# bayesiains/nflows

Hardware: AMD Instinct MI355X
Metric: log_prob samples/sec (dim=64, K=8, 32-layer RQ-NSF) + max |fwd∘inv − x| (higher is better)
Workload: dtype f32 (inputs, outputs, spline arithmetic, accumulation; conditioner GEMMs: every fp32 operand carried as 3 f16 pieces = 33 significand bits, i.e. at the reference's own fp32 operand width, 5 cross products per multiply-add -- 3 on the f16 MFMA, the 2 at the 2^-22 level from the pieces' high bytes on

## Files before the change

### include/nflows_amd.h

```cpp
#ifndef NFLOWS_AMD_H
#define NFLOWS_AMD_H

#include <stddef.h>
#include <stdint.h>

#ifdef __cplusplus
extern "C" {
#endif

#define NFA_ABI_VERSION 19

#define NFA_OK 0
#define NFA_ERR_INVALID_ARGUMENT 1
#define NFA_ERR_UNSUPPORTED 2
#define NFA_ERR_MIN_BIN_WIDTH 3
#define NFA_ERR_MIN_BIN_HEIGHT 4
#define NFA_ERR_HIP 5

#define NFA_STATUS_OUTSIDE_DOMAIN 1
#define NFA_STATUS_NEG_DISCRIMINANT 2
#define NFA_STATUS_BAD_INDEX 4

#define NFA_FLAG_INVERSE 1
#define NFA_FLAG_ACCUMULATE_LOGABSDET 2
// ... 3 lines not shown

#define NFA_FLAG_STANDARD_NORMAL_LOG_PROB 16
#define NFA_FLAG_SKIP_OUTPUTS 32

#define NFA_FLAG_RESIDUAL_BLOCKS 64
#define NFA_FLAG_PAD_COLUMNS_SHIFT 8
#define NFA_FLAG_PAD_COLUMNS_MASK 0x700
#define NFA_FLAG_PAD_COLUMNS(n) ((n) << NFA_FLAG_PAD_COLUMNS_SHIFT)
#define NFA_FLAG_ACTIVATION_SHIFT 12
#define NFA_FLAG_ACTIVATION_MASK 0x7000
#define NFA_ACTIVATION_RELU 0
#define NFA_ACTIVATION_LEAKY_RELU 1
#define NFA_ACTIVATION_ELU 2
#define NFA_ACTIVATION_TANH 3
#define NFA_FLAG_ACTIVATION(a) ((a) << NFA_FLAG_ACTIVATION_SHIFT)

#define NFA_TAILS_NONE 0
#define NFA_TAILS_LINEAR 1

#define NFA_SCALE_DEFAULT 0
#define NFA_SCALE_GENERAL 1
#define NFA_SCALE_ADDITIVE 2
#define NFA_SCALE_GIVEN 3
#define NFA_SCALE_SOFTPLUS 4

typedef struct nfa_rqs_spec {
    int32_t num_bins;
    int32_t tails;
    double left, right;
    double bottom, top;
// ... 361 lines not shown
```

### nflows_amd/_native.py

```python
import ctypes
import os

import torch

_PKG_DIR = os.path.dirname(os.path.abspath(__file__))
LIB_PATH = os.environ.get("NFLOWS_AMD_LIB") or os.path.join(_PKG_DIR, "libnflows_amd.so")

OK = 0
ERR_INVALID_ARGUMENT = 1
ERR_UNSUPPORTED = 2
ERR_MIN_BIN_WIDTH = 3
ERR_MIN_BIN_HEIGHT = 4
ERR_HIP = 5

STATUS_OUTSIDE_DOMAIN = 1
STATUS_NEG_DISCRIMINANT = 2
STATUS_BAD_INDEX = 4

FLAG_INVERSE, FLAG_ACCUMULATE_LOGABSDET, FLAG_WEIGHTS_BF16X3, FLAG_LOGITS_LOG2E = 1, 2, 4, 8
FLAG_STANDARD_NORMAL_LOG_PROB, FLAG_SKIP_OUTPUTS = 16, 32
FLAG_RESIDUAL_BLOCKS = 64
FLAG_PAD_COLUMNS_SHIFT = 8
FLAG_ACTIVATION_SHIFT = 12
ACTIVATION_RELU, ACTIVATION_LEAKY_RELU, ACTIVATION_ELU, ACTIVATION_TANH = 0, 1, 2, 3
TAILS_NONE, TAILS_LINEAR = 0, 1
NONLIN_EXP, NONLIN_TANH, NONLIN_LOG_TANH, NONLIN_LEAKY_RELU, NONLIN_SIGMOID, NONLIN_CAUCHY_CDF = 0, 1, 2, 3, 4, 5
SCALE_DEFAULT, SCALE_GENERAL, SCALE_ADDITIVE, SCALE_GIVEN, SCALE_SOFTPLUS = 0, 1, 2, 3, 4

ABI_VERSION = 19

EXPORTS = (
    "nfa_abi_version",
    "nfa_build_arch",
    "nfa_strerror",
    "nfa_last_hip_error",
    "nfa_rqs_coupling_f32",
    "nfa_rqs_coupling_backward_f32",
    "nfa_rqs_coupling_fused_linear_f32",
# ... 328 lines not shown
```

### nflows_amd/csrc/f16x3_gemm.hpp

```cpp
#pragma once

#include "bf16x3_gemm.hpp"

namespace nfa {

typedef _Float16 f16x8 __attribute__((ext_vector_type(8)));
typedef int i32x8 __attribute__((ext_vector_type(8)));

namespace k8x {

constexpr int kScaleA = 119, kScaleB = 127;

#ifdef NFA_ABL_NO_MFMA
#define NFA_K8X_F16(a, b, c) (c)
#define NFA_K8X_BF8(a, b, c) (c)
#else
#define NFA_K8X_F16(a, b, c) __builtin_amdgcn_mfma_f32_32x32x16_f16(a, b, c, 0, 0, 0)
#define NFA_K8X_BF8(a, b, c) __builtin_amdgcn_mfma_scale_f32_32x32x64_f8f6f4(a, b, c, 1, 1, 0, kScaleA, 0, kScaleB)
#endif

__device__ __forceinline__ void request_stage(WeightStream& sm) {
    const int dst_slot = sm.slot >= 1 ? sm.slot - 1 : kRing - 1;
    const char* stage = reinterpret_cast<const char*>(sm.w) + (size_t)sm.fetch * (kStageVec4 * 16);
    const __amdgpu_buffer_rsrc_t rsrc =
        __builtin_amdgcn_make_buffer_rsrc(const_cast<char*>(stage), (short)0, kStageVec4 * 16, 0x00020000);
    const int wave = __builtin_amdgcn_readfirstlane(sm.tid >> 6);
    char* slot = reinterpret_cast<char*>(sm.ring) + dst_slot * (kStageVec4 * 16) + wave * (kWave * 16);
    const unsigned lane_off = (unsigned)sm.tid * 16u;
#pragma unroll
    for (int i = 0; i < 3; ++i)
        __builtin_amdgcn_raw_ptr_buffer_load_lds(rsrc, (__attribute__((address_space(3))) void*)(slot + i * kBlock * 16), 16,
                                                 lane_off, i * kBlock * 16, 0, 0);
    sm.fetch = (sm.fetch + 1 == sm.num_stages) ? 0 : sm.fetch + 1;
}

struct Pieces {
    uvec4 h, l, r;
};

#define NFA_K8X_ASM asm volatile

#define NFA_K8X_SPLIT_REST                                                  \
    "v_fma_mixlo_f16 %1, %3, 1.0, 0 op_sel_hi:[0,0,0]\n\t"                  \
    "v_fma_mixhi_f16 %1, %4, 1.0, 0 op_sel_hi:[0,0,0]\n\t"                  \
    "v_fma_mix_f32 %3, %3, 1.0, -%1 op_sel_hi:[0,0,1]\n\t"                  \
    "v_fma_mix_f32 %4, %4, 1.0, -%1 op_sel:[0,0,1] op_sel_hi:[0,0,1]\n\t"   \
    "v_fma_mixlo_f16 %2, %3, %8, 0 op_sel_hi:[0,0,0]\n\t"                   \
    "v_fma_mixhi_f16 %2, %4, %8, 0 op_sel_hi:[0,0,0]"
// ... 78 lines not shown

__device__ __forceinline__ i32x8 join_x(vec4f lo, vec4f hi) {
    const uvec4 a = __builtin_bit_cast(uvec4, lo), b = __builtin_bit_cast(uvec4, hi);
    return i32x8{(int)a[0], (int)a[1], (int)a[2], (int)a[3], (int)b[0], (int)b[1], (int)b[2], (int)b[3]};
}

struct Lead {
    vec4f h0, l0, h1, l1;
};
__device__ __forceinline__ Lead read_lead(const vec4f* stage) {
    return Lead{stage[0 * 64], stage[1 * 64], stage[2 * 64], stage[3 * 64]};
}

#define NFA_K8X_FENCE() __builtin_amdgcn_sched_barrier(0)

template <bool LAST>
__device__ __forceinline__ void stage_kmajor(f32x16& acc0, f32x16& acc1, const Pieces& b0, const Pieces& b1, const i32x8& bx,
                                             WeightStream& sm, int lane, Lead& lead) {
    request_stage(sm);
    const vec4f* cur = sm.ring + sm.slot * kStageVec4 + lane;
    const f16x8 bh0 = __builtin_bit_cast(f16x8, b0.h), bl0 = __builtin_bit_cast(f16x8, b0.l);
    const f16x8 bh1 = __builtin_bit_cast(f16x8, b1.h), bl1 = __builtin_bit_cast(f16x8, b1.l);
    const vec4f x0l = cur[4 * 64], x0h = cur[5 * 64];
    const vec4f h0 = cur[6 * 64], l0 = cur[7 * 64], h1 = cur[8 * 64], l1 = cur[9 * 64], x1l = cur[10 * 64], x1h = cur[11 * 64];
    NFA_K8X_FENCE();
    {
        const f16x8 ah0 = __builtin_bit_cast(f16x8, lead.h0), al0 = __builtin_bit_cast(f16x8, lead.l0);
        const f16x8 ah1 = __builtin_bit_cast(f16x8, lead.h1), al1 = __builtin_bit_cast(f16x8, lead.l1);
        acc0 = NFA_K8X_F16(ah0, bl0, acc0);
        acc0 = NFA_K8X_F16(al0, bh0, acc0);
        acc0 = NFA_K8X_F16(ah0, bh0, acc0);
        acc0 = NFA_K8X_F16(ah1, bl1, acc0);
        acc0 = NFA_K8X_F16(al1, bh1, acc0);
        acc0 = NFA_K8X_F16(ah1, bh1, acc0);
        acc0 = NFA_K8X_BF8(join_x(x0l, x0h), bx, acc0);
    }
    const f16x8 ah0 = __builtin_bit_cast(f16x8, h0), al0 = __builtin_bit_cast(f16x8, l0);
    const f16x8 ah1 = __builtin_bit_cast(f16x8, h1), al1 = __builtin_bit_cast(f16x8, l1);
    const i32x8 ax = join_x(x1l, x1h);
    acc1 = NFA_K8X_F16(ah0, bl0, acc1);
    acc1 = NFA_K8X_F16(al0, bh0, acc1);
    acc1 = NFA_K8X_F16(ah0, bh0, acc1);
    NFA_K8X_FENCE();
    stream_advance(sm);
    if constexpr (!LAST) lead = read_lead(sm.ring + sm.slot * kStageVec4 + lane);
    NFA_K8X_FENCE();
    acc1 = NFA_K8X_F16(ah1, bl1, acc1);
    acc1 = NFA_K8X_F16(al1, bh1, acc1);
    acc1 = NFA_K8X_F16(ah1, bh1, acc1);
    acc1 = NFA_K8X_BF8(ax, bx, acc1);
}

template <int NKS, class PairFn>
__device__ __forceinline__ void gemm_kmajor_pairs(f32x16 (&acc)[4], WeightStream& sm, int lane, PairFn&& pair) {
    static_assert(NKS % 2 == 0, "pairs of k-steps");
    Lead lead = read_lead(sm.ring + sm.slot * kStageVec4 + lane);
#pragma unroll
    for (int pr = 0; pr < NKS / 2; ++pr) {
        Pieces b0, b1;
        pair(pr, b0, b1);
        const i32x8 bx = bf8_operand(b0, b1);
        stage_kmajor<false>(acc[0], acc[1], b0, b1, bx, sm, lane, lead);
        if (pr + 1 < NKS / 2) stage_kmajor<false>(acc[2], acc[3], b0, b1, bx, sm, lane, lead);
        else stage_kmajor<true>(acc[2], acc[3], b0, b1, bx, sm, lane, lead);
    }
}

template <int NKS>
__device__ __forceinline__ void gemm_kmajor(f32x16 (&acc)[4], const Pieces (&p)[8], WeightStream& sm, int lane) {
    gemm_kmajor_pairs<NKS>(acc, sm, lane, [&](int pr, Pieces& b0, Pieces& b1) {
        b0 = p[2 * pr];
        b1 = p[2 * pr + 1];
    });
}

__device__ __forceinline__ void gemm_kmajor_relu(f32x16 (&acc)[4], const f32x16 (&src)[4], float scale, WeightStream& sm,
                                                 int lane) {
    gemm_kmajor_pairs<8>(acc, sm, lane, [&](int pr, Pieces& b0, Pieces& b1) {
        if (pr == 0) tile_to_pieces<true, true>(src[pr], scale, b0, b1);
        else tile_to_pieces<true, false>(src[pr], scale, b0, b1);
    });
}

}
}
```

### nflows_amd/csrc/rqs_resnet_f16x3.hip

```cpp

#include "rqs_resnet_f16x3_kernel.hpp"

using namespace nfa;

static k8x::KernelFn f16x3_kernel(bool inverse, int init_ks, int K, bool dbg, bool bias_lds) {
    if (K != 8) {
        const k8x::KernelFn kern = k8x::bins_kernel_a(K, inverse, init_ks, bias_lds);
        return kern ? kern : k8x::bins_kernel_b(K, inverse, init_ks, bias_lds);
    }
    if (!bias_lds) {
        if (init_ks == 4)
            return dbg ? (inverse ? k8x::rqs_resnet_f16x3_global_bias_kernel<true, 4, true> : k8x::rqs_resnet_f16x3_global_bias_kernel<false, 4, true>)
                       : (inverse ? k8x::rqs_resnet_f16x3_global_bias_kernel<true, 4> : k8x::rqs_resnet_f16x3_global_bias_kernel<false, 4>);
        return dbg ? (inverse ? k8x::rqs_resnet_f16x3_global_bias_kernel<true, 2, true> : k8x::rqs_resnet_f16x3_global_bias_kernel<false, 2, true>)
                   : (inverse ? k8x::rqs_resnet_f16x3_global_bias_kernel<true, 2> : k8x::rqs_resnet_f16x3_global_bias_kernel<false, 2>);
    }
    if (init_ks == 4)
        return dbg ? (inverse ? k8x::rqs_resnet_f16x3_kernel<true, 4, true> : k8x::rqs_resnet_f16x3_kernel<false, 4, true>)
                   : (inverse ? k8x::rqs_resnet_f16x3_kernel<true, 4> : k8x::rqs_resnet_f16x3_kernel<false, 4>);
    return dbg ? (inverse ? k8x::rqs_resnet_f16x3_kernel<true, 2, true> : k8x::rqs_resnet_f16x3_kernel<false, 2, true>)
               : (inverse ? k8x::rqs_resnet_f16x3_kernel<true, 2> : k8x::rqs_resnet_f16x3_kernel<false, 2>);
}

static int launch_f16x3(const LayerCall& c, const float* scales, float act_scale, float* dbg_logits = nullptr) {
    int exponent = 0;
    if (!(act_scale > 0.0f) || frexpf(act_scale, &exponent) != 0.5f) return NFA_ERR_INVALID_ARGUMENT;
    k8x::Args a;
    int activation = 0;
    int rc = check_layer_call(c, {NFA_FLAG_ACTIVATION_MASK, true, false, false}, &a.sp, &activation);
    if (rc != NFA_OK) return rc;
    if (activation != NFA_ACTIVATION_RELU || (dbg_logits && a.sp.K != 8)) return NFA_ERR_UNSUPPORTED;
    if (c.batch == 0) return NFA_OK;
    if (!layer_buffers_given(c) || !c.bias || !scales || !c.redo) return NFA_ERR_INVALID_ARGUMENT;
    rc = fill_layer_args(a, c);
    if (rc != NFA_OK) return rc;
    a.act_scale = act_scale;
    a.bias = c.bias;
    a.scales = scales;
    a.tables = c.tables;
    a.redo = c.redo;
    a.dbg_logits = dbg_logits;
    const int init_ks = c.num_identity > 32 ? 4 : 2;
    const int rows_per_feature = spline_rows_per_feature(a.sp.K);
    a.num_stages = init_ks + 16 * c.num_blocks + 2 * (c.num_transform * rows_per_feature / 32);
    a.bias_per_layer = 128 + 256 * c.num_blocks + c.num_transform * rows_per_feature;
    const size_t lds_rows = (size_t)kRing * kStageVec4 * 16 + (size_t)(kBlock / kWave) * c.features * kRowPad * sizeof(float);
    const int final_floats = c.num_transform * rows_per_feature;
    const size_t lds_area = lds_rows + (size_t)k8x::bias_area_floats(c.num_blocks, final_floats) * sizeof(float);
    const size_t lds_plain = lds_rows + (size_t)final_floats * sizeof(float);
    const size_t two_per_cu = 80 * 1024 - 2048;
    const size_t launch_limit = kCuLds - 2048;
    const bool bias_lds = lds_area <= launch_limit && (dbg_logits || lds_area <= two_per_cu || lds_plain > two_per_cu);
    const size_t lds = bias_lds ? lds_area : lds_plain;
    int64_t blocks = c.batch >> 7;
    const int64_t per_cu = lds <= two_per_cu ? 2 : 1;
    const int64_t cap = (int64_t)device_cu_count() * per_cu;
    if (blocks > cap) blocks = cap;
    const bool inv = (c.flags & NFA_FLAG_INVERSE) != 0;
    const k8x::KernelFn kern = f16x3_kernel(inv, init_ks, a.sp.K, dbg_logits, bias_lds);
    if (!kern) return NFA_ERR_UNSUPPORTED;
    note_layer_kernel("k8x::rqs_resnet_f16x3_kernel<inverse=%d, init_ks=%d, K=%d, dbg=%d, bias=%s>", inv ? 1 : 0, init_ks, a.sp.K,
                      dbg_logits ? 1 : 0, bias_lds ? "lds" : "global");
    return launch_kernel(kern, dim3((unsigned)blocks), dim3(kBlock), lds, (hipStream_t)c.stream, a, kCuLds - 2048);
}

extern "C" int nfa_rqs_flow_resnet_f16x3_f32(const float* inputs, const void* weights_packed, const float* bias_packed,
                                             const float* scales, const int32_t* flow_tables, int32_t num_layers,
                                             float* outputs, float* logabsdet, int32_t* redo_blocks, int32_t* status,
                                             int64_t batch, int32_t features, int32_t num_transform,
                                             int32_t num_identity, int32_t hidden_features, int32_t num_blocks,
                                             float act_scale, const nfa_rqs_spec* spec, int32_t flags, void* stream) {
    return launch_f16x3({inputs, weights_packed, bias_packed, flow_tables, num_layers, outputs, logabsdet, redo_blocks,
                         status, batch, features, num_transform, num_identity, hidden_features, num_blocks, spec, flags,
// ... 19 lines not shown
```

### nflows_amd/csrc/rqs_resnet_f16x3_kernel.hpp

```cpp
#pragma once

#include "f16x3_gemm.hpp"
#include "rqs_resnet_f16_kernel.hpp"

#include <hip/hip_ext.h>
#include <stdlib.h>
#include <type_traits>

namespace nfa {
namespace k8x {

struct Args {
    const float* x;
    const vec4f* w;
    const float* bias;
    const float* scales;
    const int32_t* tables;
    float* out;
    float* lad;
    int32_t* redo;
    int32_t* status;
    int64_t batch;
    int D, dt, di, num_blocks, num_layers, num_stages, bias_per_layer, accumulate;
    RqsDev sp;
// ... 81 lines not shown
        k8h::spline_seq_range<MASK, (U0 * N) / 32, (U1 * N) / 32>(f, sp);
    }
};

#define NFA_K8X_PUMP_F16(U, A_, B_)                                         \
    acc = NFA_K8X_F16(A_, B_, acc);                                         \
    __builtin_amdgcn_sched_barrier(0);                                      \
    w.template span<(U), (U) + 1>();                                        \
    __builtin_amdgcn_sched_barrier(0)
#define NFA_K8X_PUMP_BF8(U, A_, B_)                                         \
    acc = NFA_K8X_BF8(A_, B_, acc);                                         \
    __builtin_amdgcn_sched_barrier(0);                                      \
    w.template span<(U), (U) + 2>();                                        \
    __builtin_amdgcn_sched_barrier(0)

template <int HS, class W>
__device__ __forceinline__ void stage_pumped(f32x16& acc, const Pieces (&p)[8], const i32x8 (&bx)[4], WeightStream& sm, int lane,
                                             Lead& lead, W& w) {
    request_stage(sm);
    const vec4f* cur = sm.ring + sm.slot * kStageVec4 + lane;
    vec4f xa = cur[8 * 64], xb = cur[9 * 64];
    vec4f fh0 = lead.h0, fl0 = lead.l0, fh1 = lead.h1, fl1 = lead.l1;
    {
        const Pieces& b0 = p[HS * 4 + 0];
        const Pieces& b1 = p[HS * 4 + 1];
        const f16x8 bh0 = __builtin_bit_cast(f16x8, b0.h), bl0 = __builtin_bit_cast(f16x8, b0.l);
        const f16x8 bh1 = __builtin_bit_cast(f16x8, b1.h), bl1 = __builtin_bit_cast(f16x8, b1.l);
        const f16x8 ah0 = __builtin_bit_cast(f16x8, fh0), al0 = __builtin_bit_cast(f16x8, fl0);
        const f16x8 ah1 = __builtin_bit_cast(f16x8, fh1), al1 = __builtin_bit_cast(f16x8, fl1);
        const i32x8 ax = join_x(xa, xb);
        NFA_K8X_PUMP_F16(HS * 16 + 0, ah0, bl0);
        NFA_K8X_PUMP_F16(HS * 16 + 1, al0, bh0);
        NFA_K8X_PUMP_F16(HS * 16 + 2, ah0, bh0);
        fh0 = cur[4 * 64];
// ... 9 lines not shown
    }
    {
        const Pieces& b0 = p[HS * 4 + 2];
        const Pieces& b1 = p[HS * 4 + 3];
        const f16x8 bh0 = __builtin_bit_cast(f16x8, b0.h), bl0 = __builtin_bit_cast(f16x8, b0.l);
        const f16x8 bh1 = __builtin_bit_cast(f16x8, b1.h), bl1 = __builtin_bit_cast(f16x8, b1.l);
        const f16x8 ah0 = __builtin_bit_cast(f16x8, fh0), al0 = __builtin_bit_cast(f16x8, fl0);
        const f16x8 ah1 = __builtin_bit_cast(f16x8, fh1), al1 = __builtin_bit_cast(f16x8, fl1);
        const i32x8 ax = join_x(xa, xb);
        NFA_K8X_PUMP_F16(HS * 16 + 8, ah0, bl0);
        NFA_K8X_PUMP_F16(HS * 16 + 9, al0, bh0);
        NFA_K8X_PUMP_F16(HS * 16 + 10, ah0, bh0);
        NFA_K8X_PUMP_F16(HS * 16 + 11, ah1, bl1);
        NFA_K8X_PUMP_F16(HS * 16 + 12, al1, bh1);
        NFA_K8X_PUMP_F16(HS * 16 + 13, ah1, bh1);
        stream_advance(sm);
        lead = read_lead(sm.ring + sm.slot * kStageVec4 + lane);
        __builtin_amdgcn_sched_barrier(0);
        NFA_K8X_PUMP_BF8(HS * 16 + 14, ax, bx[HS * 2 + 1]);
    }
}
#undef NFA_K8X_PUMP_F16
#undef NFA_K8X_PUMP_BF8

template <class W>
__device__ __forceinline__ void gemm_tile_pumped(f32x16& acc, const Pieces (&p)[8], const i32x8 (&bx)[4], WeightStream& sm, int lane,
                                                 Lead& lead, W&& w) {
    stage_pumped<0>(acc, p, bx, sm, lane, lead, w);
    stage_pumped<1>(acc, p, bx, sm, lane, lead, w);
}

template <int TI, int T, int KB, class Steps, class BiasPtr>
__device__ __forceinline__ void any_group_tiles(f32x16& acc, Steps& f, BiasPtr gb, const Pieces (&p)[8], const i32x8 (&bx)[4],
                                                WeightStream& sm, int lane, Lead& lead, const RqsDev& sp) {
    if constexpr (TI < T) {
        constexpr int kMask = k8h::any_tile_mask(KB, TI);
        load_bias_tile(acc, gb + TI * 32);
        if constexpr (kMask != 0) gemm_tile_pumped(acc, p, bx, sm, lane, lead, SeqWeave<kMask, Steps>{f, sp});
        else gemm_tile_pumped(acc, p, bx, sm, lane, lead, NoWeave{});
        k8h::take_chunk<TI, KB>(f, acc);
        any_group_tiles<TI + 1, T, KB, Steps, BiasPtr>(acc, f, gb, p, bx, sm, lane, lead, sp);
    }
}

__device__ __forceinline__ bool not_finite(float v) { return !(__builtin_fabsf(v) < INFINITY); }

template <bool INVERSE, int INIT_KS, bool DBG, int KB, bool BIAS_LDS>
__device__ __forceinline__ void rqs_resnet_f16x3_body(const Args& a) {
    static_assert(!DBG || KB == 8, "the diagnostic instances: 8 bins");
    constexpr int kFinalRows = KB == 8 ? 24 : 16 * ((3 * KB - 1 + 15) / 16);
    constexpr int NW = kBlock / kWave;
    extern __shared__ __attribute__((aligned(16))) float lds_dyn[];
    __shared__ int s_tab[2][kTabLayer];
    __shared__ int s_final[128];
    __shared__ int s_bad[NW];
    const int tid = threadIdx.x, lane = tid & 63, wave = __builtin_amdgcn_readfirstlane(tid >> 6);
    const int D = a.D, dt = a.dt;
    int my_status = 0;
    auto checked = [&](int v, bool used) {
        my_status |= (used && (v < 0 || v >= D)) ? NFA_STATUS_BAD_INDEX : 0;
        return v < 0 ? 0 : (v >= D ? D - 1 : v);
    };
    const int te = tid & (kTabLayer - 1);
    s_tab[0][te] = checked(a.tables[te], te < kTabTr ? te < a.di : te - kTabTr < dt);
    s_final[te] = checked(a.tables[a.num_layers * kTabLayer + te], te < D);

    WeightStream sm;
    sm.w = a.w;
    sm.ring = reinterpret_cast<vec4f*>(lds_dyn);
    sm.slot = 1;
    sm.fetch = 0;
    sm.num_stages = a.num_stages * a.num_layers;
    sm.tid = tid;
    lds_f32* s_area = (lds_f32*)lds_dyn + kRing * kStageVec4 * 4 + NW * D * kRowPad;
    lds_f32* s_traw = s_area + bias_area_hidden_floats(a.num_blocks);
    auto request_hidden = [&](int layer) {
        const float* src = a.bias + (size_t)layer * a.bias_per_layer;
        const int bytes = bias_area_hidden_floats(a.num_blocks) * 4;
        if (wave >= 2) bias_area_piece<4>(src, bytes, (wave - 2) * 256, s_area + (wave - 2) * 64);
        for (int j = wave; j < a.num_blocks; j += NW) bias_area_piece<16>(src, bytes, 512 + j * 1024, s_area + 128 + j * 256);
    };
    if constexpr (BIAS_LDS) request_hidden(0);
    request_stage(sm);
    sm.slot = 2;
    request_stage(sm);
    sm.slot = 0;
    asm volatile("s_waitcnt vmcnt(0)" ::: "memory");
    __syncthreads();

#ifdef NFA_K8X_STAGGER
    if (blockIdx.x >= (gridDim.x >> 1))
        for (int i = 0; i < NFA_K8X_STAGGER; ++i) __builtin_amdgcn_s_sleep(127);
#endif
    lds_f32* s_row = (lds_f32*)lds_dyn + kRing * kStageVec4 * 4 + wave * D * kRowPad;
    lds_f32* s_fbias = BIAS_LDS ? s_traw + kTabLayer : s_area;
    auto request_final = [&](int layer) {
        const float* src = a.bias + (size_t)layer * a.bias_per_layer + bias_area_hidden_floats(a.num_blocks);
        const int bytes = dt * kFinalRows * 4;
        for (int j = wave; j * 1024 < bytes; j += NW) bias_area_piece<16>(src, bytes, j * 1024, s_fbias + j * 256);
    };
    auto request_table = [&](int layer) {
        if (wave < 2) bias_area_piece<4>(a.tables + layer * kTabLayer, kTabLayer * 4, wave * 256, s_traw + wave * 64);
    };
    const int groups = dt >> 2;
    const int64_t num_quads = a.batch >> 7;
    const int gemms = 2 + 2 * a.num_blocks;
    const float S = a.act_scale;
    int tb = 0;

    for (int64_t quad = blockIdx.x; quad < num_quads; quad += gridDim.x) {
        const int64_t row0 = (quad << 7) + (wave << 5);
        int lane_here = lane, di = a.di;
        asm volatile("" : "+v"(lane_here), "+s"(di));
        const int half = lane_here >> 5, r = lane_here & 31;
        {
            const vec4f* xv = reinterpret_cast<const vec4f*>(a.x + row0 * D);
            const int nvec = D * 8;
            for (int e0 = lane; e0 < nvec; e0 += kWave * 4) {
                vec4f v[4];
#pragma unroll
                for (int u = 0; u < 4; ++u) {
                    const int e = e0 + u * kWave;
                    v[u] = xv[e < nvec ? e : 0];
                }
#pragma unroll
                for (int u = 0; u < 4; ++u) {
// ... 2 lines not shown
                        const int rr = (e * 4) / D, c0 = e * 4 - rr * D;
                        s_row[(c0 + 0) * kRowPad + rr] = v[u].x;
                        s_row[(c0 + 1) * kRowPad + rr] = v[u].y;
                        s_row[(c0 + 2) * kRowPad + rr] = v[u].z;
                        s_row[(c0 + 3) * kRowPad + rr] = v[u].w;
                    }
                }
            }
        }
        __builtin_amdgcn_fence(__ATOMIC_RELEASE, "wavefront");
        __builtin_amdgcn_fence(__ATOMIC_ACQUIRE, "wavefront");

        float lad_acc = 0.0f;
        int quad_status = 0;
        for (int layer = 0; layer < a.num_layers; ++layer) {
            if ((layer + (blockIdx.x >= (gridDim.x >> 1) ? 1 : 0)) & 1) __builtin_amdgcn_s_setprio(1);
            else __builtin_amdgcn_s_setprio(0);
            const int* tab = s_tab[tb];
            const int nl = layer + 1 < a.num_layers ? layer + 1 : 0;
            if constexpr (!BIAS_LDS) {
                unsigned all = ~0u;
                asm volatile("" : "+s"(all));
                const int te_l = (int)__builtin_amdgcn_mbcnt_hi(all, __builtin_amdgcn_mbcnt_lo(all, 0u)) + ((wave & 1) << 6);
                s_tab[tb ^ 1][te_l] = checked(a.tables[nl * kTabLayer + te_l], te_l < kTabTr ? te_l < a.di : te_l - kTabTr < dt);
            }
            if constexpr (BIAS_LDS) {
                request_final(layer);
                request_table(nl);
                __builtin_amdgcn_sched_barrier(0);
            }
            std::conditional_t<BIAS_LDS, const lds_f32*, const float*> bias;
            if constexpr (BIAS_LDS) bias = s_area + half * 16;
// ... 10 lines not shown
                    v0 = i0 < di ? v0 : 0.0f;
                    v1 = i0 + 1 < di ? v1 : 0.0f;
                    unsigned hi, lo, rr;
                    split3_scaled(v0, v1, S, hi, lo, rr);
                    p[ks].h[j2] = hi;
                    p[ks].l[j2] = lo;
                    p[ks].r[j2] = rr;
                }
            }

            f32x16 h[4];
            float hs;
            {
#pragma unroll
                for (int t = 0; t < 4; ++t) load_bias_tile(h[t], bias + t * 32);
                gemm_kmajor<INIT_KS>(h, p, sm, lane);
                float s0[2];
                uniform_load(sc, s0);
                hs = s0[0];
            }
            bias += 128;
            sc += 2;
            if constexpr (BIAS_LDS) {
                unsigned all = ~0u;
                asm volatile("" : "+s"(all));
                const int te_l = (int)__builtin_amdgcn_mbcnt_hi(all, __builtin_amdgcn_mbcnt_lo(all, 0u)) + ((wave & 1) << 6);
                s_tab[tb ^ 1][te_l] = checked(((const lds_i32*)s_traw)[te_l], te_l < kTabTr ? te_l < a.di : te_l - kTabTr < dt);
            } else {
                const float* fbias = a.bias + (size_t)layer * a.bias_per_layer + 128 + 256 * a.num_blocks;
                for (int i = tid; i < dt * kFinalRows; i += kBlock) s_fbias[i] = fbias[i];
                if (a.num_blocks == 0) __syncthreads();
            }

            for (int blk = 0; blk < a.num_blocks; ++blk) {
                float sb[4];
                f32x16 u[4];
#pragma unroll
                for (int t = 0; t < 4; ++t) load_bias_tile(u[t], bias + t * 32);
                gemm_kmajor_relu(u, h, hs, sm, lane);
                uniform_load(sc, sb);
                const float skip = hs * sb[3];
#pragma unroll
                for (int t = 0; t < 4; ++t) {
                    f32x16 b1;
                    load_bias_tile(b1, bias + 128 + t * 32);
#pragma unroll
                    for (int q_ = 0; q_ < 16; ++q_) h[t][q_] = __builtin_fmaf(h[t][q_], skip, b1[q_]);
                }
                gemm_kmajor_relu(h, u, sb[0], sm, lane);
                hs = sb[2];
                bias += 256;
                sc += 4;
            }

            if constexpr (BIAS_LDS) {
                request_hidden(nl);
                __builtin_amdgcn_sched_barrier(0);
            }
#pragma unroll
            for (int t = 0; t < 4; ++t) tile_to_pieces<false>(h[t], hs, p[2 * t], p[2 * t + 1]);

            if constexpr (KB == 8) {
                using Steps = FusedSteps<INVERSE, 8>;
                Steps fa{}, fb{};
// ... 21 lines not shown
                            float* dst = a.dbg_logits + (size_t)(row0 + r) * (dt * kFinalRows) + tile * 32 + half * 16;
#pragma unroll
                            for (int q_ = 0; q_ < 16; ++q_) dst[q_] = t[q_] * kappa;
                            asm volatile("s_waitcnt vmcnt(0)" ::: "memory");
                        }
                    }
                };
                UnitWeave<k8h::kUnitNumA, Steps> w0{fa, fb, a.sp};
                UnitWeave<k8h::kUnitFinishA, Steps> w1{fa, fb, a.sp};
                UnitWeave<k8h::kUnitFinishB, Steps> w2{fa, fb, a.sp};
                for (int g = 0; g < groups; ++g) {
                    lds_f32* slot0 = s_row + tab[kTabTr + g * 4 + half * 2] * kRowPad + r;
                    lds_f32* slot1 = s_row + tab[kTabTr + g * 4 + half * 2 + 1] * kRowPad + r;
                    load_bias_tile(acc[0], fbias + (g * 3 + 0) * 32);
                    if (g > 0) {
                        gemm_tile_pumped(acc[0], p, bx, sm, lane, lead, w2);
                        commit(fb, slot_b);
                    } else {
                        gemm_tile_pumped(acc[0], p, bx, sm, lane, lead, NoWeave{});
                    }
                    store_logits(acc[0], g * 3 + 0);
                    fa.x = *slot0;
#pragma unroll
                    for (int j = 0; j < 8; ++j) {
                        fa.ew[j] = acc[0][j];
                        fa.eh[j] = acc[0][8 + j];
                    }
                    load_bias_tile(acc[1], fbias + (g * 3 + 1) * 32);
                    gemm_tile_pumped(acc[1], p, bx, sm, lane, lead, w0);
                    store_logits(acc[1], g * 3 + 1);
                    fb.x = *slot1;
#pragma unroll
                    for (int j = 0; j < 8; ++j) {
                        if (j < 7) fa.sd[j] = acc[1][j];
                        fb.ew[j] = acc[1][8 + j];
                    }
                    load_bias_tile(acc[2], fbias + (g * 3 + 2) * 32);
                    gemm_tile_pumped(acc[2], p, bx, sm, lane, lead, w1);
                    store_logits(acc[2], g * 3 + 2);
                    commit(fa, slot0);
#pragma unroll
                    for (int j = 0; j < 8; ++j) {
                        fb.eh[j] = acc[2][j];
                        if (j < 7) fb.sd[j] = acc[2][8 + j];
                    }
                    slot_b = slot1;
                }
                k8h::spline_unit_range<k8h::kUnitFinishB, 0, k8h::spline_unit_slices<k8h::kUnitFinishB, Steps>()>(fa, fb, a.sp);
                commit(fb, slot_b);
            }
            else {
                constexpr int T = kFinalRows / 16;
                static_assert(T >= 1 && T <= 6, "2 .. 32 bins");
// ... 37 lines not shown
            }
            tb ^= 1;
            __builtin_amdgcn_fence(__ATOMIC_RELEASE, "wavefront");
            __builtin_amdgcn_fence(__ATOMIC_ACQUIRE, "wavefront");
        }

        lad_acc += __shfl_xor(lad_acc, 32, kWave);
        const float sumsq = tile_row_sumsq((const float*)s_row, a.Ds, half, r);
        const bool bad = not_finite(lad_acc) || not_finite(sumsq);
        const bool wave_bad = __builtin_amdgcn_ballot_w64(bad) != 0;
        if (lane == 0) s_bad[wave] = wave_bad ? 1 : 0;
        asm volatile("s_waitcnt vmcnt(0)" ::: "memory");
        __syncthreads();
        int any_bad = 0;
#pragma unroll
        for (int w_ = 0; w_ < NW; ++w_) any_bad |= s_bad[w_];
        if (!any_bad) {
            if (!a.skip_out) {
                vec4f* ov = reinterpret_cast<vec4f*>(a.out + row0 * D);
                const int nvec = D * 8;
                for (int e = lane; e < nvec; e += kWave) {
                    const int rr = (e * 4) / D, c0 = e * 4 - rr * D;
                    vec4f v;
                    v.x = s_row[s_final[c0 + 0] * kRowPad + rr];
                    v.y = s_row[s_final[c0 + 1] * kRowPad + rr];
                    v.z = s_row[s_final[c0 + 2] * kRowPad + rr];
                    v.w = s_row[s_final[c0 + 3] * kRowPad + rr];
                    ov[e] = v;
                }
            }
            if (half == 0) {
                float* dst = a.lad + row0 + r;
                float v = a.accumulate ? *dst + lad_acc : lad_acc;
                if (a.normal) v = (-0.5f * sumsq - a.log_z) + v;
                *dst = v;
            }
            my_status |= quad_status;
        }
        if (tid == 0) a.redo[quad] = any_bad ? 1 : 0;
        asm volatile("s_waitcnt vmcnt(0)" ::: "memory");
        __syncthreads();
    }
    asm volatile("s_waitcnt vmcnt(0)" ::: "memory");
    if (my_status && a.status) atomicOr(a.status, my_status);
}

template <bool INVERSE, int INIT_KS, bool DBG = false, int KB = 8>
__global__ void __launch_bounds__(kBlock, 2) rqs_resnet_f16x3_kernel(const Args a) {
    rqs_resnet_f16x3_body<INVERSE, INIT_KS, DBG, KB, true>(a);
}
template <bool INVERSE, int INIT_KS, bool DBG = false, int KB = 8>
__global__ void __launch_bounds__(kBlock, 2) rqs_resnet_f16x3_global_bias_kernel(const Args a) {
    rqs_resnet_f16x3_body<INVERSE, INIT_KS, DBG, KB, false>(a);
}

}
}


namespace nfa {
namespace k8x {
typedef void (*KernelFn)(const Args);
KernelFn bins_kernel_a(int K, bool inverse, int init_ks, bool bias_lds);
KernelFn bins_kernel_b(int K, bool inverse, int init_ks, bool bias_lds);
}
}
```

### nflows_amd/ops.py

```python
import ctypes
import math
import os

import numpy as np
import torch

from . import _native as N
from . import autograd as AG
from .errors import InputOutsideDomain

_status_words = {}
_error_mode = "deferred"
_launch_hook = None


_last_redo = None


def last_redo_blocks():
    return None if _last_redo is None else int((_last_redo != 0).sum().item())


def set_launch_hook(hook):
    global _launch_hook
# ... 2045 lines not shown


_ACTIVATION_CODES = {id(torch.nn.functional.relu): N.ACTIVATION_RELU, id(torch.relu): N.ACTIVATION_RELU,
                     id(torch.nn.functional.leaky_relu): N.ACTIVATION_LEAKY_RELU, id(torch.nn.functional.elu): N.ACTIVATION_ELU,
                     id(torch.tanh): N.ACTIVATION_TANH, id(torch.nn.functional.tanh): N.ACTIVATION_TANH}


def activation_code(fn):
    return _ACTIVATION_CODES.get(id(fn))


K8S_ENABLED = os.environ.get("NFA_K8S", "1") != "0"
K8S_ALWAYS = os.environ.get("NFA_K8S", "1") == "2"
K8C_ENABLED = os.environ.get("NFA_K8C", "1") != "0"
K8C_ALWAYS = os.environ.get("NFA_K8C", "1") == "2"
_cu_counts = {}


def use_tile16(batch, num_bins, context, device, activation=0):
    if not K8S_ENABLED or num_bins != 8 or context is not None or activation != N.ACTIVATION_RELU:
        return 0
    if capture_last_layer_logits.active is not None:
        return 0
    key = device.index if device.index is not None else torch.cuda.current_device()
    cus = _cu_counts.get(key)
    if cus is None:
        cus = _cu_counts[key] = torch.cuda.get_device_properties(key).multi_processor_count
    if K8C_ENABLED and capture_last_layer_bins.active is None and (K8C_ALWAYS or (batch + 95) // 96 <= cus):
        return 2
    return 1 if (K8S_ALWAYS or (batch + 127) // 128 <= cus) else 0
# ... 189 lines not shown
    def finish(self, redo):
        self.logits = unpack_last_layer_logits(self._packed, self._dt)
        self.redo = redo


def rqs_coupling_resnet_f16x3(inputs, packed_f16x3, packed_exact, tables, num_transform, num_identity, num_blocks,
                              spec, inverse=False, accumulate_into=None, num_layers=1,
                              standard_normal_log_prob=False, pad=None, act_scale=K8X_ACT_SCALE):
    weights, biases, scales = packed_f16x3

    def launch(x, ctx, out, lad, redo, flags, status, stream):
        lib = N.load()
        B, D = x.shape
        args = (N.ptr(x), N.ptr(weights), N.ptr(biases), N.ptr(scales), N.ptr(tables), num_layers, N.ptr(out),
                N.ptr(lad), N.ptr(redo), status, B, D, num_transform, num_identity, 128, num_blocks,
                float(act_scale), ctypes.byref(spec), flags, stream)
        capture = capture_last_layer_logits.active
        if capture is None:
            return lib.nfa_rqs_flow_resnet_f16x3_f32(*args)
        rc = lib.nfa_rqs_flow_resnet_f16x3_logits_f32(*args, N.ptr(capture.buffer(B, num_transform, x.device)))
        if rc == N.OK:
            capture.finish(redo)
        return rc
    return _whole_layer_launch(launch, inputs, inverse, accumulate_into, standard_normal_log_prob, pad, spec=spec,
                               redo=(*packed_exact, tables, num_layers, num_transform, num_identity, num_blocks))


def rqs_coupling_fused_linear(inputs, hidden, weight_packed, bias_padded, transform_idx, spec,
                              inverse=False, in_perm=None, out_scatter=None, accumulate_into=None):
    N.require_device_f32("inputs", inputs, 2)
    N.require_device_f32("hidden", hidden, 2)
# ... 29 lines not shown
```

Baseline: 26.74 million.

## Add wide 8-wave k8x resnet kernel sharing one weight stream across two quads

Adds a wide form of the f16x3 resnet flow kernel with 512 threads (8 waves) per block. Each block processes two 128-row quads at once, and both halves share a double-width LDS weight ring, so every streamed weight stage is fetched once for two quads instead of once per block. The form is chosen automatically when the batch is large enough (at least 2 blocks per CU), with an environment and flag override. The cost is double the LDS ring size, one block per CU, barriers that now span 8 waves, and predicated handling of an odd trailing quad.

```diff
diff --git a/include/nflows_amd.h b/include/nflows_amd.h
--- a/include/nflows_amd.h
+++ b/include/nflows_amd.h
@@ -41,6 +41,12 @@
 #define NFA_ACTIVATION_ELU 2
 #define NFA_ACTIVATION_TANH 3
 #define NFA_FLAG_ACTIVATION(a) ((a) << NFA_FLAG_ACTIVATION_SHIFT)
+#define NFA_FLAG_K8X_FORM_SHIFT 16
+#define NFA_FLAG_K8X_FORM_MASK 0x30000
+#define NFA_K8X_FORM_AUTO 0
+#define NFA_K8X_FORM_NARROW 1
+#define NFA_K8X_FORM_WIDE 2
+#define NFA_FLAG_K8X_FORM(f) ((f) << NFA_FLAG_K8X_FORM_SHIFT)
 
 #define NFA_TAILS_NONE 0
 #define NFA_TAILS_LINEAR 1
diff --git a/nflows_amd/_native.py b/nflows_amd/_native.py
--- a/nflows_amd/_native.py
+++ b/nflows_amd/_native.py
@@ -22,6 +22,7 @@
 FLAG_RESIDUAL_BLOCKS = 64
 FLAG_PAD_COLUMNS_SHIFT = 8
 FLAG_ACTIVATION_SHIFT = 12
+FLAG_K8X_FORM_SHIFT = 16
 ACTIVATION_RELU, ACTIVATION_LEAKY_RELU, ACTIVATION_ELU, ACTIVATION_TANH = 0, 1, 2, 3
 TAILS_NONE, TAILS_LINEAR = 0, 1
 NONLIN_EXP, NONLIN_TANH, NONLIN_LOG_TANH, NONLIN_LEAKY_RELU, NONLIN_SIGMOID, NONLIN_CAUCHY_CDF = 0, 1, 2, 3, 4, 5
diff --git a/nflows_amd/csrc/f16x3_gemm.hpp b/nflows_amd/csrc/f16x3_gemm.hpp
--- a/nflows_amd/csrc/f16x3_gemm.hpp
+++ b/nflows_amd/csrc/f16x3_gemm.hpp
@@ -32,6 +32,36 @@
         __builtin_amdgcn_raw_ptr_buffer_load_lds(rsrc, (__attribute__((address_space(3))) void*)(slot + i * kBlock * 16), 16,
                                                  lane_off, i * kBlock * 16, 0, 0);
     sm.fetch = (sm.fetch + 1 == sm.num_stages) ? 0 : sm.fetch + 1;
+}
+
+template <int WAVES, int SUB>
+__device__ __forceinline__ void request_stage(WeightStream& sm) {
+    static_assert(WAVES == 4 || WAVES == 8, "narrow or wide");
+    if constexpr (WAVES == 4) {
+        request_stage(sm);
+    } else if constexpr (SUB == 0) {
+        const int dst_half = sm.slot >= 2 ? sm.slot - 2 : sm.slot + 2 * kRing - 2;
+        const char* stage = reinterpret_cast<const char*>(sm.w) + (size_t)sm.fetch * (kStageVec4 * 16);
+        const __amdgpu_buffer_rsrc_t rsrc =
+            __builtin_amdgcn_make_buffer_rsrc(const_cast<char*>(stage), (short)0, 2 * kStageVec4 * 16, 0x00020000);
+        const int wave = __builtin_amdgcn_readfirstlane(sm.tid >> 6);
+        char* slot = reinterpret_cast<char*>(sm.ring) + dst_half * (kStageVec4 * 16) + wave * (kWave * 16);
+        const unsigned lane_off = (unsigned)sm.tid * 16u;
+#pragma unroll
+        for (int i = 0; i < 3; ++i)
+            __builtin_amdgcn_raw_ptr_buffer_load_lds(rsrc, (__attribute__((address_space(3))) void*)(slot + i * WAVES * kWave * 16),
+                                                     16, lane_off, i * WAVES * kWave * 16, 0, 0);
+        sm.fetch = (sm.fetch + 2 == sm.num_stages) ? 0 : sm.fetch + 2;
+    }
+}
+template <int WAVES, int SUB>
+__device__ __forceinline__ void stream_advance(WeightStream& sm) {
+    if constexpr (WAVES == 4) {
+        stream_advance(sm);
+    } else {
+        if constexpr (SUB == 1) asm volatile("s_waitcnt vmcnt(3)\n\ts_waitcnt lgkmcnt(0)\n\ts_barrier" ::: "memory");
+        sm.slot = (sm.slot + 1 == 2 * kRing) ? 0 : sm.slot + 1;
+    }
 }
 
 struct Pieces {
@@ -140,10 +170,10 @@
 
 #define NFA_K8X_FENCE() __builtin_amdgcn_sched_barrier(0)
 
-template <bool LAST>
+template <bool LAST, int WAVES = 4, int SUB = 0>
 __device__ __forceinline__ void stage_kmajor(f32x16& acc0, f32x16& acc1, const Pieces& b0, const Pieces& b1, const i32x8& bx,
                                              WeightStream& sm, int lane, Lead& lead) {
-    request_stage(sm);
+    request_stage<WAVES, SUB>(sm);
     const vec4f* cur = sm.ring + sm.slot * kStageVec4 + lane;
     const f16x8 bh0 = __builtin_bit_cast(f16x8, b0.h), bl0 = __builtin_bit_cast(f16x8, b0.l);
     const f16x8 bh1 = __builtin_bit_cast(f16x8, b1.h), bl1 = __builtin_bit_cast(f16x8, b1.l);
@@ -168,7 +198,7 @@
     acc1 = NFA_K8X_F16(al0, bh0, acc1);
     acc1 = NFA_K8X_F16(ah0, bh0, acc1);
     NFA_K8X_FENCE();
-    stream_advance(sm);
+    stream_advance<WAVES, SUB>(sm);
     if constexpr (!LAST) lead = read_lead(sm.ring + sm.slot * kStageVec4 + lane);
     NFA_K8X_FENCE();
     acc1 = NFA_K8X_F16(ah1, bl1, acc1);
@@ -177,7 +207,7 @@
     acc1 = NFA_K8X_BF8(ax, bx, acc1);
 }
 
-template <int NKS, class PairFn>
+template <int NKS, int WAVES, class PairFn>
 __device__ __forceinline__ void gemm_kmajor_pairs(f32x16 (&acc)[4], WeightStream& sm, int lane, PairFn&& pair) {
     static_assert(NKS % 2 == 0, "pairs of k-steps");
     Lead lead = read_lead(sm.ring + sm.slot * kStageVec4 + lane);
@@ -186,23 +216,24 @@
         Pieces b0, b1;
         pair(pr, b0, b1);
         const i32x8 bx = bf8_operand(b0, b1);
-        stage_kmajor<false>(acc[0], acc[1], b0, b1, bx, sm, lane, lead);
-        if (pr + 1 < NKS / 2) stage_kmajor<false>(acc[2], acc[3], b0, b1, bx, sm, lane, lead);
-        else stage_kmajor<true>(acc[2], acc[3], b0, b1, bx, sm, lane, lead);
-    }
-}
-
-template <int NKS>
+        stage_kmajor<false, WAVES, 0>(acc[0], acc[1], b0, b1, bx, sm, lane, lead);
+        if (pr + 1 < NKS / 2) stage_kmajor<false, WAVES, 1>(acc[2], acc[3], b0, b1, bx, sm, lane, lead);
+        else stage_kmajor<true, WAVES, 1>(acc[2], acc[3], b0, b1, bx, sm, lane, lead);
+    }
+}
+
+template <int NKS, int WAVES = 4>
 __device__ __forceinline__ void gemm_kmajor(f32x16 (&acc)[4], const Pieces (&p)[8], WeightStream& sm, int lane) {
-    gemm_kmajor_pairs<NKS>(acc, sm, lane, [&](int pr, Pieces& b0, Pieces& b1) {
+    gemm_kmajor_pairs<NKS, WAVES>(acc, sm, lane, [&](int pr, Pieces& b0, Pieces& b1) {
         b0 = p[2 * pr];
         b1 = p[2 * pr + 1];
     });
 }
 
+template <int WAVES = 4>
 __device__ __forceinline__ void gemm_kmajor_relu(f32x16 (&acc)[4], const f32x16 (&src)[4], float scale, WeightStream& sm,
                                                  int lane) {
-    gemm_kmajor_pairs<8>(acc, sm, lane, [&](int pr, Pieces& b0, Pieces& b1) {
+    gemm_kmajor_pairs<8, WAVES>(acc, sm, lane, [&](int pr, Pieces& b0, Pieces& b1) {
         if (pr == 0) tile_to_pieces<true, true>(src[pr], scale, b0, b1);
         else tile_to_pieces<true, false>(src[pr], scale, b0, b1);
     });
diff --git a/nflows_amd/csrc/rqs_resnet_f16x3.hip b/nflows_amd/csrc/rqs_resnet_f16x3.hip
--- a/nflows_amd/csrc/rqs_resnet_f16x3.hip
+++ b/nflows_amd/csrc/rqs_resnet_f16x3.hip
@@ -22,13 +22,20 @@
                : (inverse ? k8x::rqs_resnet_f16x3_kernel<true, 2> : k8x::rqs_resnet_f16x3_kernel<false, 2>);
 }
 
+static k8x::KernelFn f16x3_wide_kernel(bool inverse, int init_ks) {
+    if (init_ks == 4) return inverse ? k8x::rqs_resnet_f16x3_kernel_wide<true, 4> : k8x::rqs_resnet_f16x3_kernel_wide<false, 4>;
+    return inverse ? k8x::rqs_resnet_f16x3_kernel_wide<true, 2> : k8x::rqs_resnet_f16x3_kernel_wide<false, 2>;
+}
+
 static int launch_f16x3(const LayerCall& c, const float* scales, float act_scale, float* dbg_logits = nullptr) {
     int exponent = 0;
     if (!(act_scale > 0.0f) || frexpf(act_scale, &exponent) != 0.5f) return NFA_ERR_INVALID_ARGUMENT;
     k8x::Args a;
     int activation = 0;
-    int rc = check_layer_call(c, {NFA_FLAG_ACTIVATION_MASK, true, false, false}, &a.sp, &activation);
+    int rc = check_layer_call(c, {NFA_FLAG_ACTIVATION_MASK | NFA_FLAG_K8X_FORM_MASK, true, false, false}, &a.sp, &activation);
     if (rc != NFA_OK) return rc;
+    const int form = (c.flags & NFA_FLAG_K8X_FORM_MASK) >> NFA_FLAG_K8X_FORM_SHIFT;
+    if (form > NFA_K8X_FORM_WIDE) return NFA_ERR_INVALID_ARGUMENT;
     if (activation != NFA_ACTIVATION_RELU || (dbg_logits && a.sp.K != 8)) return NFA_ERR_UNSUPPORTED;
     if (c.batch == 0) return NFA_OK;
     if (!layer_buffers_given(c) || !c.bias || !scales || !c.redo) return NFA_ERR_INVALID_ARGUMENT;
@@ -53,10 +60,22 @@
     const bool bias_lds = lds_area <= launch_limit && (dbg_logits || lds_area <= two_per_cu || lds_plain > two_per_cu);
     const size_t lds = bias_lds ? lds_area : lds_plain;
     int64_t blocks = c.batch >> 7;
+    const bool inv = (c.flags & NFA_FLAG_INVERSE) != 0;
+    const size_t lds_wide = 2 * lds_rows + (size_t)k8x::bias_area_floats(c.num_blocks, final_floats) * sizeof(float);
+    const bool wide_fits = a.sp.K == 8 && !dbg_logits && lds_wide <= launch_limit;
+    const bool wide = wide_fits && form != NFA_K8X_FORM_NARROW &&
+                      (form == NFA_K8X_FORM_WIDE || blocks >= (int64_t)k8x::kWideBlocksPerCu * device_cu_count());
+    if (wide) {
+        int64_t grid = (blocks + 1) >> 1;
+        if (grid > device_cu_count()) grid = device_cu_count();
+        note_layer_kernel("k8x::rqs_resnet_f16x3_kernel<inverse=%d, init_ks=%d, K=%d, dbg=0, waves=8, bias=lds>", inv ? 1 : 0, init_ks,
+                          a.sp.K);
+        return launch_kernel(f16x3_wide_kernel(inv, init_ks), dim3((unsigned)grid), dim3(2 * kBlock), lds_wide, (hipStream_t)c.stream,
+                             a, kCuLds - 2048);
+    }
     const int64_t per_cu = lds <= two_per_cu ? 2 : 1;
     const int64_t cap = (int64_t)device_cu_count() * per_cu;
     if (blocks > cap) blocks = cap;
-    const bool inv = (c.flags & NFA_FLAG_INVERSE) != 0;
     const k8x::KernelFn kern = f16x3_kernel(inv, init_ks, a.sp.K, dbg_logits, bias_lds);
     if (!kern) return NFA_ERR_UNSUPPORTED;
     note_layer_kernel("k8x::rqs_resnet_f16x3_kernel<inverse=%d, init_ks=%d, K=%d, dbg=%d, bias=%s>", inv ? 1 : 0, init_ks, a.sp.K,
diff --git a/nflows_amd/csrc/rqs_resnet_f16x3_kernel.hpp b/nflows_amd/csrc/rqs_resnet_f16x3_kernel.hpp
--- a/nflows_amd/csrc/rqs_resnet_f16x3_kernel.hpp
+++ b/nflows_amd/csrc/rqs_resnet_f16x3_kernel.hpp
@@ -119,10 +119,10 @@
     w.template span<(U), (U) + 2>();                                        \
     __builtin_amdgcn_sched_barrier(0)
 
-template <int HS, class W>
+template <int HS, int WAVES, class W>
 __device__ __forceinline__ void stage_pumped(f32x16& acc, const Pieces (&p)[8], const i32x8 (&bx)[4], WeightStream& sm, int lane,
                                              Lead& lead, W& w) {
-    request_stage(sm);
+    request_stage<WAVES, HS>(sm);
     const vec4f* cur = sm.ring + sm.slot * kStageVec4 + lane;
     vec4f xa = cur[8 * 64], xb = cur[9 * 64];
     vec4f fh0 = lead.h0, fl0 = lead.l0, fh1 = lead.h1, fl1 = lead.l1;
@@ -162,7 +162,7 @@
         NFA_K8X_PUMP_F16(HS * 16 + 11, ah1, bl1);
         NFA_K8X_PUMP_F16(HS * 16 + 12, al1, bh1);
         NFA_K8X_PUMP_F16(HS * 16 + 13, ah1, bh1);
-        stream_advance(sm);
+        stream_advance<WAVES, HS>(sm);
         lead = read_lead(sm.ring + sm.slot * kStageVec4 + lane);
         __builtin_amdgcn_sched_barrier(0);
         NFA_K8X_PUMP_BF8(HS * 16 + 14, ax, bx[HS * 2 + 1]);
@@ -171,11 +171,11 @@
 #undef NFA_K8X_PUMP_F16
 #undef NFA_K8X_PUMP_BF8
 
-template <class W>
+template <int WAVES = 4, class W>
 __device__ __forceinline__ void gemm_tile_pumped(f32x16& acc, const Pieces (&p)[8], const i32x8 (&bx)[4], WeightStream& sm, int lane,
                                                  Lead& lead, W&& w) {
-    stage_pumped<0>(acc, p, bx, sm, lane, lead, w);
-    stage_pumped<1>(acc, p, bx, sm, lane, lead, w);
+    stage_pumped<0, WAVES>(acc, p, bx, sm, lane, lead, w);
+    stage_pumped<1, WAVES>(acc, p, bx, sm, lane, lead, w);
 }
 
 template <int TI, int T, int KB, class Steps, class BiasPtr>
@@ -193,11 +193,14 @@
 
 __device__ __forceinline__ bool not_finite(float v) { return !(__builtin_fabsf(v) < INFINITY); }
 
-template <bool INVERSE, int INIT_KS, bool DBG, int KB, bool BIAS_LDS>
+template <bool INVERSE, int INIT_KS, bool DBG, int KB, bool BIAS_LDS, int WAVES = 4>
 __device__ __forceinline__ void rqs_resnet_f16x3_body(const Args& a) {
     static_assert(!DBG || KB == 8, "the diagnostic instances: 8 bins");
+    constexpr bool WIDE = WAVES == 8;
+    static_assert(WAVES == 4 || (WIDE && KB == 8 && BIAS_LDS && !DBG), "the wide form: 8 bins, bias area, no diagnostics");
+    constexpr int kRingFloats = kRing * kStageVec4 * 4 * (WIDE ? 2 : 1);
     constexpr int kFinalRows = KB == 8 ? 24 : 16 * ((3 * KB - 1 + 15) / 16);
-    constexpr int NW = kBlock / kWave;
+    constexpr int NW = WAVES;
     extern __shared__ __attribute__((aligned(16))) float lds_dyn[];
     __shared__ int s_tab[2][kTabLayer];
     __shared__ int s_final[128];
@@ -220,18 +223,25 @@
     sm.fetch = 0;
     sm.num_stages = a.num_stages * a.num_layers;
     sm.tid = tid;
-    lds_f32* s_area = (lds_f32*)lds_dyn + kRing * kStageVec4 * 4 + NW * D * kRowPad;
+    lds_f32* s_area = (lds_f32*)lds_dyn + kRingFloats + NW * D * kRowPad;
     lds_f32* s_traw = s_area + bias_area_hidden_floats(a.num_blocks);
     auto request_hidden = [&](int layer) {
         const float* src = a.bias + (size_t)layer * a.bias_per_layer;
         const int bytes = bias_area_hidden_floats(a.num_blocks) * 4;
-        if (wave >= 2) bias_area_piece<4>(src, bytes, (wave - 2) * 256, s_area + (wave - 2) * 64);
+        if (wave >= NW - 2) bias_area_piece<4>(src, bytes, (wave - (NW - 2)) * 256, s_area + (wave - (NW - 2)) * 64);
         for (int j = wave; j < a.num_blocks; j += NW) bias_area_piece<16>(src, bytes, 512 + j * 1024, s_area + 128 + j * 256);
     };
     if constexpr (BIAS_LDS) request_hidden(0);
-    request_stage(sm);
-    sm.slot = 2;
-    request_stage(sm);
+    if constexpr (WIDE) {
+        sm.slot = 2;
+        request_stage<WAVES, 0>(sm);
+        sm.slot = 4;
+        request_stage<WAVES, 0>(sm);
+    } else {
+        request_stage(sm);
+        sm.slot = 2;
+        request_stage(sm);
+    }
     sm.slot = 0;
     asm volatile("s_waitcnt vmcnt(0)" ::: "memory");
     __syncthreads();
@@ -240,7 +250,7 @@
     if (blockIdx.x >= (gridDim.x >> 1))
         for (int i = 0; i < NFA_K8X_STAGGER; ++i) __builtin_amdgcn_s_sleep(127);
 #endif
-    lds_f32* s_row = (lds_f32*)lds_dyn + kRing * kStageVec4 * 4 + wave * D * kRowPad;
+    lds_f32* s_row = (lds_f32*)lds_dyn + kRingFloats + wave * D * kRowPad;
     lds_f32* s_fbias = BIAS_LDS ? s_traw + kTabLayer : s_area;
     auto request_final = [&](int layer) {
         const float* src = a.bias + (size_t)layer * a.bias_per_layer + bias_area_hidden_floats(a.num_blocks);
@@ -256,8 +266,13 @@
     const float S = a.act_scale;
     int tb = 0;
 
-    for (int64_t quad = blockIdx.x; quad < num_quads; quad += gridDim.x) {
-        const int64_t row0 = (quad << 7) + (wave << 5);
+    const int64_t num_passes = WIDE ? (num_quads + 1) >> 1 : num_quads;
+    for (int64_t pass = blockIdx.x; pass < num_passes; pass += gridDim.x) {
+        const int64_t quad_mine = WIDE ? 2 * pass + (wave >> 2) : pass;
+        const int live_bit = WIDE ? (int)(((uint64_t)quad_mine - (uint64_t)num_quads) >> 63) : 1;
+        const bool live = live_bit != 0;
+        const int64_t quad = quad_mine - 1 + live_bit;
+        const int64_t row0 = (quad << 7) + ((WIDE ? wave & 3 : wave) << 5);
         int lane_here = lane, di = a.di;
         asm volatile("" : "+v"(lane_here), "+s"(di));
         const int half = lane_here >> 5, r = lane_here & 31;
@@ -290,8 +305,13 @@
         float lad_acc = 0.0f;
         int quad_status = 0;
         for (int layer = 0; layer < a.num_layers; ++layer) {
-            if ((layer + (blockIdx.x >= (gridDim.x >> 1) ? 1 : 0)) & 1) __builtin_amdgcn_s_setprio(1);
-            else __builtin_amdgcn_s_setprio(0);
+#ifdef NFA_K8X_WIDE_NOPRIO
+            if constexpr (!WIDE)
+#endif
+            {
+                if ((layer + ((WIDE ? wave >= 4 : blockIdx.x >= (gridDim.x >> 1)) ? 1 : 0)) & 1) __builtin_amdgcn_s_setprio(1);
+                else __builtin_amdgcn_s_setprio(0);
+            }
             const int* tab = s_tab[tb];
             const int nl = layer + 1 < a.num_layers ? layer + 1 : 0;
             if constexpr (!BIAS_LDS) {
@@ -332,7 +352,7 @@
             {
 #pragma unroll
                 for (int t = 0; t < 4; ++t) load_bias_tile(h[t], bias + t * 32);
-                gemm_kmajor<INIT_KS>(h, p, sm, lane);
+                gemm_kmajor<INIT_KS, WAVES>(h, p, sm, lane);
                 float s0[2];
                 uniform_load(sc, s0);
                 hs = s0[0];
@@ -355,7 +375,7 @@
                 f32x16 u[4];
 #pragma unroll
                 for (int t = 0; t < 4; ++t) load_bias_tile(u[t], bias + t * 32);
-                gemm_kmajor_relu(u, h, hs, sm, lane);
+                gemm_kmajor_relu<WAVES>(u, h, hs, sm, lane);
                 uniform_load(sc, sb);
                 const float skip = hs * sb[3];
 #pragma unroll
@@ -365,7 +385,7 @@
 #pragma unroll
                     for (int q_ = 0; q_ < 16; ++q_) h[t][q_] = __builtin_fmaf(h[t][q_], skip, b1[q_]);
                 }
-                gemm_kmajor_relu(h, u, sb[0], sm, lane);
+                gemm_kmajor_relu<WAVES>(h, u, sb[0], sm, lane);
                 hs = sb[2];
                 bias += 256;
                 sc += 4;
@@ -417,10 +437,10 @@
                     lds_f32* slot1 = s_row + tab[kTabTr + g * 4 + half * 2 + 1] * kRowPad + r;
                     load_bias_tile(acc[0], fbias + (g * 3 + 0) * 32);
                     if (g > 0) {
-                        gemm_tile_pumped(acc[0], p, bx, sm, lane, lead, w2);
+                        gemm_tile_pumped<WAVES>(acc[0], p, bx, sm, lane, lead, w2);
                         commit(fb, slot_b);
                     } else {
-                        gemm_tile_pumped(acc[0], p, bx, sm, lane, lead, NoWeave{});
+                        gemm_tile_pumped<WAVES>(acc[0], p, bx, sm, lane, lead, NoWeave{});
                     }
                     store_logits(acc[0], g * 3 + 0);
                     fa.x = *slot0;
@@ -430,7 +450,7 @@
                         fa.eh[j] = acc[0][8 + j];
                     }
                     load_bias_tile(acc[1], fbias + (g * 3 + 1) * 32);
-                    gemm_tile_pumped(acc[1], p, bx, sm, lane, lead, w0);
+                    gemm_tile_pumped<WAVES>(acc[1], p, bx, sm, lane, lead, w0);
                     store_logits(acc[1], g * 3 + 1);
                     fb.x = *slot1;
 #pragma unroll
@@ -439,7 +459,7 @@
                         fb.ew[j] = acc[1][8 + j];
                     }
                     load_bias_tile(acc[2], fbias + (g * 3 + 2) * 32);
-                    gemm_tile_pumped(acc[2], p, bx, sm, lane, lead, w1);
+                    gemm_tile_pumped<WAVES>(acc[2], p, bx, sm, lane, lead, w1);
                     store_logits(acc[2], g * 3 + 2);
                     commit(fa, slot0);
 #pragma unroll
@@ -507,8 +527,8 @@
         __syncthreads();
         int any_bad = 0;
 #pragma unroll
-        for (int w_ = 0; w_ < NW; ++w_) any_bad |= s_bad[w_];
-        if (!any_bad) {
+        for (int w_ = 0; w_ < 4; ++w_) any_bad |= s_bad[(WIDE ? wave & 4 : 0) + w_];
+        if (!any_bad && live) {
             if (!a.skip_out) {
                 vec4f* ov = reinterpret_cast<vec4f*>(a.out + row0 * D);
                 const int nvec = D * 8;
@@ -530,7 +550,7 @@
             }
             my_status |= quad_status;
         }
-        if (tid == 0) a.redo[quad] = any_bad ? 1 : 0;
+        if ((WIDE ? (tid & 255) == 0 && live : tid == 0)) a.redo[quad] = any_bad ? 1 : 0;
         asm volatile("s_waitcnt vmcnt(0)" ::: "memory");
         __syncthreads();
     }
@@ -545,6 +565,13 @@
 template <bool INVERSE, int INIT_KS, bool DBG = false, int KB = 8>
 __global__ void __launch_bounds__(kBlock, 2) rqs_resnet_f16x3_global_bias_kernel(const Args a) {
     rqs_resnet_f16x3_body<INVERSE, INIT_KS, DBG, KB, false>(a);
+}
+
+constexpr int kWideBlocksPerCu = 2;
+
+template <bool INVERSE, int INIT_KS>
+__global__ void __launch_bounds__(2 * kBlock, 1) rqs_resnet_f16x3_kernel_wide(const Args a) {
+    rqs_resnet_f16x3_body<INVERSE, INIT_KS, false, 8, true, 8>(a);
 }
 
 }
diff --git a/nflows_amd/ops.py b/nflows_amd/ops.py
--- a/nflows_amd/ops.py
+++ b/nflows_amd/ops.py
@@ -2083,6 +2083,8 @@
 K8S_ALWAYS = os.environ.get("NFA_K8S", "1") == "2"
 K8C_ENABLED = os.environ.get("NFA_K8C", "1") != "0"
 K8C_ALWAYS = os.environ.get("NFA_K8C", "1") == "2"
+K8X_FORMS = {"auto": 0, "narrow": 1, "wide": 2}
+K8X_FORM = K8X_FORMS[os.environ.get("NFA_K8X_FORM", "auto")]
 _cu_counts = {}
 
 
@@ -2302,7 +2304,7 @@
         B, D = x.shape
         args = (N.ptr(x), N.ptr(weights), N.ptr(biases), N.ptr(scales), N.ptr(tables), num_layers, N.ptr(out),
                 N.ptr(lad), N.ptr(redo), status, B, D, num_transform, num_identity, 128, num_blocks,
-                float(act_scale), ctypes.byref(spec), flags, stream)
+                float(act_scale), ctypes.byref(spec), flags | K8X_FORM << N.FLAG_K8X_FORM_SHIFT, stream)
         capture = capture_last_layer_logits.active
         if capture is None:
             return lib.nfa_rqs_flow_resnet_f16x3_f32(*args)
```

New measurement: 28.08 million (median of 6 runs). 5.0% higher.
